# YXHXianYu/RVCP-Real-Time-Path-Tracer

Hardware: AMD Instinct MI355X
Metric: Msamples/sec (pixels*SPP/s) + frame ms, Cornell Box 1024^2 SPP=30 (higher is better)
Workload: dtype f32

## Files before the change

### rvcp-real-time-path-tracer_amd/csrc/rvcp_host.cpp

```cpp
#include <dlfcn.h>
#include <hip/hip_runtime.h>
#include <rccl/rccl.h>

#include <atomic>
#include <cfloat>
#include <cmath>
#include <cstdio>
#include <cstdlib>
#include <chrono>
#include <condition_variable>
#include <cstring>
#include <memory>
#include <exception>
#include <initializer_list>
#include <mutex>
#include <new>
#include <string>
#include <thread>
#include <vector>

#include "../../include/rvcp.h"
#include "rvcp_internal.h"
#include "rvcp_frame_plan.h"
#include "rvcp_jit.h"
// ... 84 lines not shown
        int bvh = 0;
    } capacity[2][2];
    int legacy_capacity = 0;
    uint32_t n_simds = 1024;

    TriRecord *d_tri = nullptr;
    rvcp_face_t *d_faces = nullptr;
    rvcp_vertex_t *d_verts = nullptr;
    MatRecord *d_mats = nullptr;
    FaceShade *d_shade = nullptr;
    LightRecord *d_lights = nullptr;
    rvcp_material_t *d_rawmats = nullptr;
    rvcp_sphere_t *d_spheres = nullptr;
    Bvh4Node *d_bvh_nodes = nullptr;
    TriRecord *d_bvh_tris = nullptr;
    int32_t bvh_root = 0;
    uint32_t bvh_n4 = 0;
    uint32_t bvh_slots = 0;
    int bvh_depth = 0;
    uint32_t bvh_prefix = 0;
    float *d_gamma = nullptr;
    float *d_unorm = nullptr;
    unsigned long long *d_counters = nullptr;
    uint32_t n_faces = 0, n_lights = 0, n_mats = 0, n_verts = 0, n_spheres = 0;
    bool lights_same = false;
    bool rcp_fast = false;
    bool has_metal = false;
    std::shared_ptr<JitKernels> jit[2];
    std::string jit_err;
    int32_t sampling = RVCP_SAMPLING_UNIFORM;
    int32_t jit_sampling[2] = {RVCP_SAMPLING_UNIFORM, -1};
    std::vector<TriRecord> jit_tri;
    bool jit_bvh = false;
    float light_total = 0.0f, light_pdf = 0.0f;
    bool has_scene = false;

    SurfRecord *d_surf = nullptr;
    size_t cap_surf = 0;
    float *d_acc = nullptr;
    size_t cap_acc = 0;
    float *d_cams = nullptr, *h_cams = nullptr;
    uint32_t cap_cams = 0;

    uint32_t *d_rgba = nullptr;
    float *d_lin = nullptr;
    size_t cap_rgba = 0, cap_lin = 0;
    uint32_t *d_pack_rgba = nullptr;
    float *d_pack_lin = nullptr;
    size_t cap_surf_pack = 0;

    Stage stage[N_STAGES];

    float *d_dn[2] = {nullptr, nullptr};
    size_t cap_dn[2] = {0, 0};
    void *d_gbuf = nullptr;
    float *d_dn_in = nullptr, *d_dn_out = nullptr;
    size_t cap_gbuf = 0, cap_dn_in = 0, cap_dn_out = 0;

    float *d_tp_lin[2] = {nullptr, nullptr};
    uint32_t *d_tp_len[2] = {nullptr, nullptr};
    void *d_tp_gbuf[2] = {nullptr, nullptr};
    float *d_tp_cur = nullptr, *d_tp_show = nullptr;
    size_t cap_tp = 0, cap_tp_show = 0;
    History tp_hist;

    float *d_sv_var[2] = {nullptr, nullptr}, *d_sv_tmp[2] = {nullptr, nullptr};
// ... 783 lines not shown
        ctx->bvh_prefix = K;
        if (depth >= kBvhStack) return fail(ctx, RVCP_E_UNSUPPORTED, "BVH deeper than the traversal stack");
        const size_t S = order.size();
        if (S >= (size_t(1) << 26))
            return fail(ctx, RVCP_E_UNSUPPORTED, "BVH leaf slots exceed 2^26 (mesh too large for the leaf encoding)");
        std::vector<TriRecord> btri((10 * S * 4 + sizeof(TriRecord) - 1) / sizeof(TriRecord) + 1);
        float *packed = reinterpret_cast<float *>(btri.data());
        for (size_t j = 0; j < S; j++) {
            if (order[j] == kBvhPadId) continue;
            std::memcpy(packed + 10 * j, &tri[order[j]], 9 * sizeof(float));
            std::memcpy(packed + 10 * j + 9, &order[j], 4);
        }
        ctx->bvh_slots = 0;
        std::vector<Bvh4Node> nodes4;
        int32_t root4 = 0;
        if (bvh4_collapse(nodes, root, nodes4, root4) > kBvhStack)
            return fail(ctx, RVCP_E_UNSUPPORTED, "BVH traversal stack bound exceeded");
        std::vector<Bvh4QNode> q4;
        bvh4_quantize(nodes4, q4);
        std::vector<Bvh4Node> qbuf((q4.size() * sizeof(Bvh4QNode) + sizeof(Bvh4Node) - 1) / sizeof(Bvh4Node));
        if (!q4.empty()) std::memcpy(static_cast<void *>(qbuf.data()), q4.data(), q4.size() * sizeof(Bvh4QNode));
        ctx->bvh_n4 = 0;
        if ((rc = dev_upload<Bvh4Node>(ctx, &ctx->d_bvh_nodes, qbuf.data(), qbuf.size())) ||
            (rc = dev_upload<TriRecord>(ctx, &ctx->d_bvh_tris, btri.data(), btri.size())))
            return rc;
        ctx->bvh_root = root4;
        ctx->bvh_depth = depth;
    }
    ctx->jit[0].reset();
    ctx->jit[1].reset();
    ctx->jit_err.clear();
    ctx->jit_tri.clear();
    ctx->jit_bvh = false;
    ctx->jit_sampling[0] = ctx->sampling;
    ctx->jit_sampling[1] = -1;
    if (bvh_jit) {
        ctx->jit[0] = bvh_jit;
        ctx->jit_tri.assign(tri.begin(), tri.begin() + ctx->bvh_prefix);
        ctx->jit_bvh = true;
    }
    if (ctx->cfg.specialize == RVCP_SPECIALIZE_AUTO && ctx->cfg.accel == RVCP_ACCEL_NONE &&
        n_faces >= 1 && n_faces <= kJitMaxFaces && jit_scene_in_range(tri.data(), n_faces) &&
        !RVCP_KNOB("RVCP_NO_SPECIALIZE")) {
        const bool legacy = ctx->cfg.integrator == RVCP_INTEGRATOR_LEGACY;
        JitSpec spec;
        spec.legacy = legacy;
        spec.sphereless = n_spheres == 0;
        spec.lds_fits = n_spheres <= 64 && n_materials <= 64;
        spec.sampling = ctx->sampling;
        spec.spheres = spheres;
        spec.n_spheres = n_spheres;
        spec.n_materials = n_materials;
        ctx->jit[0] = jit_path_kernels(ctx->device, tri.data(), n_faces, spec, ctx->jit_err);
        HIP_TRY(ctx, hipSetDevice(ctx->device));
        if (!legacy) ctx->jit_tri = tri;
    }
    ctx->rcp_fast = scan_rcp_fast_scene(tri.data(), n_faces);
    ctx->n_faces = n_faces;
    ctx->n_verts = n_vertices;
    ctx->n_mats = n_materials;
    ctx->has_metal = false;
    for (uint32_t i = 0; i < n_materials; i++)
        if (materials[i].ty == 1u) ctx->has_metal = true;
    ctx->n_lights = n_lum_face_ids;
    ctx->lights_same = n_lum_face_ids >= 1;
    for (uint32_t i = 1; i < n_lum_face_ids; i++)
        if (tab.lights[i].face != tab.lights[0].face) ctx->lights_same = false;
    ctx->light_total = total;
    ctx->light_pdf = 1.0f / total;
    ctx->h_rawmats.assign(materials, materials + n_materials);
    ctx->has_scene = true;
    return RVCP_OK;
}

static int impl_upload_scene_file(rvcp_ctx_t *ctx, const char *path, rvcp_camera_t *out_camera)
{
    if (!ctx) return RVCP_E_INVALID;
    SceneFile sf;
    std::string err;
    if (read_scene_file(path, sf, err) != RVCP_OK) return fail(ctx, RVCP_E_INVALID, err);
    const rvcp_lengths_t &L = sf.lengths;
    const int rc = rvcp_upload_scene(ctx, sf.materials.data(), L.materials_len, sf.vertices.data(),
                                     L.vertices_len, sf.faces.data(), L.faces_len, sf.spheres.data(),
                                     L.spheres_len, sf.lum_face_ids.data(), L.luminous_face_id_len,
                                     sf.lum_sphere_ids.data(), L.luminous_sphere_id_len);
    if (rc == RVCP_OK && out_camera) *out_camera = sf.camera;
    return rc;
}

uint32_t rvcp_shard_rows(uint32_t height, uint32_t shard_index, uint32_t shard_count)
{
    if (shard_count == 0 || shard_index >= shard_count) return 0;
    const uint32_t stripes = (height + 7) / 8;
    uint32_t rows = 0;
    for (uint32_t s = shard_index; s < stripes; s += shard_count)
        rows += (s + 1) * 8 <= height ? 8 : height - s * 8;
    return rows;
}

static void jit_for_render(rvcp_ctx_t *ctx, bool map)
{
    ctx->jit_sampling[map] = ctx->sampling;
    if (ctx->jit_tri.empty()) return;
    std::shared_ptr<JitKernels> &jit = ctx->jit[map];
    jit.reset();
    std::string map_err;
    if (!map) ctx->jit_err.clear();
    JitSpec spec;
    spec.bvh = ctx->jit_bvh;
    spec.sampling = ctx->sampling;
    spec.spp_map = map;
    jit = jit_path_kernels(ctx->device, ctx->jit_tri.data(), (uint32_t)ctx->jit_tri.size(), spec,
                           map ? map_err : ctx->jit_err);
    (void)hipSetDevice(ctx->device);
    if (ctx->jit_bvh && jit && (!jit->bvh_path || !jit->bvh_primary)) jit.reset();
}

static FramePlanIn frame_plan_input(const rvcp_ctx_t *ctx, uint32_t n_frames, uint32_t frame_px,
                                    uint32_t stride, uint32_t spp_hint = 0)
{
    const bool cosine = ctx->sampling == RVCP_SAMPLING_COSINE;
    const bool map = spp_hint > 0;
    FramePlanIn in;
    in.integrator = ctx->cfg.integrator;
    in.kernel_variant = ctx->cfg.kernel_variant;
    in.accel = ctx->cfg.accel;
    in.spp = map ? spp_hint : ctx->cfg.spp;
    in.max_bounces = ctx->cfg.max_bounces;
    in.attenuation_stop_eps = ctx->cfg.attenuation_stop_eps;
    in.ray_t_min = ctx->cfg.ray_t_min;
    in.grid_waves_per_simd = ctx->cfg.grid_waves_per_simd;
    in.n_faces = ctx->n_faces;
    in.bvh_prefix = ctx->bvh_prefix;
    in.n_simds = ctx->n_simds;
    const rvcp_ctx::Capacity &cap = ctx->capacity[cosine][map];
    std::memcpy(in.grid_capacity, cap.grid, sizeof(in.grid_capacity));
    in.bvh_capacity = cap.bvh;
    in.legacy_capacity = ctx->legacy_capacity;
    if (const JitKernels *jk = ctx->jit[map].get()) {
        in.module = true;
        in.blocks_per_cu5 = jk->blocks_per_cu5;
        in.blocks_per_cu6 = jk->blocks_per_cu6;
        in.blocks_per_cu_bvh = jk->blocks_per_cu_bvh;
        in.blocks_per_cu_legacy = jk->blocks_per_cu_legacy;
// ... 2999 lines not shown
```

### rvcp-real-time-path-tracer_amd/csrc/rvcp_jit.cpp

```cpp
#include <hip/hip_runtime.h>

#include <dlfcn.h>
#include <sys/stat.h>
#include <unistd.h>

#include <algorithm>
#include <atomic>
#include <cerrno>
#include <cmath>
#include <cstdint>
#include <cstdio>
#include <cstdlib>
#include <cstring>
#include <list>
#include <memory>
#include <mutex>
#include <map>
#include <string>
#include <vector>

#include "rvcp_internal.h"
#include "rvcp_jit.h"
#include "build/rvcp_jit_src.h"

// ... 307 lines not shown
        decl += "    const bool " + pm.name + " = (" + t + " >= tmin) & (" + t + " <= bt" + R + ");\n";
    }
    add(pm.name);
    if (defer) {
        const std::string c = g.prefix + "c";
        accept += "        " + c + " = " + cond + ";\n";
        (inner ? *inner : decl) += "    bool " + c + ";\n";
        pm.pending.emplace_back(c, index);
        return true;
    }
    if (!pm.pending.empty()) {
        const std::string c = g.prefix + "c";
        std::string any = c, best = "best" + R;
        for (const auto &pc : pm.pending) {
            any += " | " + pc.first;
            best = "(" + pc.first + " ? " + std::to_string(pc.second) + " : " + best + ")";
        }
        accept += "        const bool " + c + " = " + cond + ";\n";
        accept += "        if (" + any + ") bt" + R + " = " + t + ";\n";
        if (R != "A")
            accept += "        best" + R + " = " + c + " ? " + std::to_string(index) + " : " + best + ";\n";
        pm.pending.clear();
        return true;
    }
    if (R == "A")
        accept += "        if (" + cond + ") btA = " + t + ";\n";
    else
        accept += "        if (" + cond + ") { bt" + R + " = " + t + "; best" + R + " = " +
                  std::to_string(index) + "; }\n";
    return true;
}

void emit_scan(std::string &out, const TriRecord *tri, uint32_t n, const char *const *rays,
               int n_rays, unsigned opts = 0)
{
    const bool skip_b = (opts & kScanSkipB) != 0, eager = (opts & kScanEagerSplit) != 0;
    const uint32_t N = n * (uint32_t)n_rays;
    std::vector<char> used(N), reused(N);
    {
        std::map<std::string, std::string> seen;
        std::map<std::string, RangeMask> prev;
        for (uint32_t u = 0; u < N; u++) {
            std::string decl, accept;
            bool ru = false;
            used[u] = emit_triangle(decl, accept, tri[u / (uint32_t)n_rays], u / (uint32_t)n_rays,
                                    rays[u % (uint32_t)n_rays], seen, prev, &ru);
            reused[u] = used[u] && ru;
        }
    }
    std::map<std::string, std::string> seen;
    std::map<std::string, RangeMask> prev;
    auto next_used = [&](uint32_t u) {
        uint32_t v = u + (uint32_t)n_rays;
        while (v < N && !used[v]) v += (uint32_t)n_rays;
        return v;
    };
    auto defers = [&](uint32_t u) {
        const uint32_t v = next_used(u);
        return used[u] && v < N && reused[v];
    };
    auto emit_plain = [&](uint32_t u) {
        std::string decl, accept;
        const std::string R(rays[u % (uint32_t)n_rays]);
        const bool defer = defers(u);
        emit_triangle(decl, accept, tri[u / (uint32_t)n_rays], u / (uint32_t)n_rays, R.c_str(),
                      seen, prev, nullptr, defer);
        out += decl;
        if (!used[u]) return;
        out += "    {\n" + accept + "    }\n";
        if (defer) return;
        out += R == "A" ? "    RVCP_SPEC_COMMIT1(btA);\n"
                        : "    RVCP_SPEC_COMMIT(bt" + R + ", best" + R + ");\n";
    };
    if (n_rays == 1) {
        for (uint32_t u = 0; u < N; u++) emit_plain(u);
        return;
    }
    auto emit_split_run = [&](const std::vector<uint32_t> &run, const char *R) {
        std::map<std::string, std::string> inner_seen;
        std::string head, body, accept;
        for (size_t k = 0; k < run.size(); k++) {
            const uint32_t u = run[k];
            const bool defer = k + 1 < run.size();
            std::string decl, inner, acc;
            if (k == 0) {
                emit_triangle(decl, acc, tri[u / 2], u / 2, R, seen, prev, nullptr, defer,
                              &inner, &inner_seen, eager);
                head += decl;
                body += inner;
            } else {
                emit_triangle(decl, acc, tri[u / 2], u / 2, R, inner_seen, prev, nullptr, defer);
                body += decl;
            }
            accept += acc;
        }
        const std::string &mask = prev[R].name;
        const std::string r(R);
        out += head;
        out += "    if (RVCP_SPEC_ANY(" + mask + ")) {\n" + body + "    {\n" + accept + "    }\n    }\n";
        out += r == "A" ? "    RVCP_SPEC_COMMIT1(btA);\n" : "    RVCP_SPEC_COMMIT(bt" + r + ", best" + r + ");\n";
    };
    for (uint32_t i = 0; i < n;) {
        const uint32_t uA = 2 * i;
        if (!used[uA]) {
            emit_plain(uA);
            emit_plain(uA + 1);
            i += 1;
            continue;
        }
        std::vector<uint32_t> run = {uA};
        while (defers(run.back())) run.push_back(next_used(run.back()));
        emit_split_run(run, "A");
        if (skip_b) {
            std::vector<uint32_t> runB;
            for (uint32_t u : run) runB.push_back(u + 1);
            emit_split_run(runB, "B");
        } else {
            for (uint32_t u : run) emit_plain(u + 1);
        }
        i = run.back() / 2 + 1;
    }
}

}
// ... 61 lines not shown
        }
        g.cross(d, e2, s1);
        for (int k = 0; k < 3; k++)
            if (s1[k].kind != Val::kZero && s1[k].mag > 126) return false;
        const Val den = g.dot(s1, e1);
        if (den.kind == Val::kZero) continue;
        if (den.grain == kNoGrain || den.grain < -126 || den.mag > 126) return false;
    }
    return true;
}

bool jit_scene_in_range(const TriRecord *tri, uint32_t n)
{
    for (uint32_t i = 0; i < n; i++)
        for (int k = 0; k < 3; k++)
            if (!(std::fabs(tri[i].v0[k]) <= 0x1p40f) || !(std::fabs(tri[i].e1[k]) <= 0x1p41f) ||
                !(std::fabs(tri[i].e2[k]) <= 0x1p41f))
                return false;
    return true;
}

std::string jit_scan_source(const TriRecord *tri, uint32_t n, unsigned opts)
{
    std::string out = "// generated by rvcp_jit.cpp: the scan of DESIGN.md §4.7 over " +
                      std::to_string(n) + " triangles\n";
    out += "__device__ __forceinline__ void spec_scan1(f3 o, f3 d, float tmin, float &bt, "
           "int &best) {\n";
    static const char *const one[] = {""}, *const two[] = {"A", "B"};
    emit_scan(out, tri, n, one, 1);
    out += "}\n";
    out += "__device__ __forceinline__ void spec_scan2(f3 oA, f3 dA, f3 oB, f3 dB, float tmin, "
           "float &btA, float &btB, int &bestB) {\n";
    emit_scan(out, tri, n, two, 2, opts);
    out += "}\n";
    return out;
}

std::string jit_sphere_source(const rvcp_sphere_t *sph, uint32_t n)
{
    if (n == 0 || n > kJitMaxSpheres || !sph) return std::string();
    std::string out = "// the scene's " + std::to_string(n) + " spheres (rvcp_jit.cpp jit_sphere_source)\n"
                      "#define RVCP_SPEC_SPHERES(X)";
    for (uint32_t i = 0; i < n; i++) {
        out += " \\\n    X(" + std::to_string(i);
        for (float v : {sph[i].center[0], sph[i].center[1], sph[i].center[2], sph[i].radius})
            out += ", " + lit_text(v);
        out += ")";
    }
    return out + "\n";
}

std::string jit_legacy_lds_source(uint32_t n_faces, uint32_t n_spheres, uint32_t n_materials)
{
    auto at_least_1 = [](uint32_t v) { return std::to_string(v ? v : 1u); };
    std::string out = "#define RVCP_LDS_FACES " + at_least_1(n_faces) + "\n#define RVCP_LDS_SPHERES " +
                      at_least_1(n_spheres) + "\n#define RVCP_LDS_MATS " + at_least_1(n_materials) + "\n";
#ifndef RVCP_NO_LDS_PRIMARY
    out += "#define RVCP_LEGACY_LDS_PRIMARY 1\n";
#endif
    return out;
}

namespace {

}

// ... 264 lines not shown
        api.log_size(prog, &ls);
        std::string log(ls, '\0');
        if (ls) api.log(prog, &log[0]);
        err = "hipRTC compile failed: " + log.substr(0, 4000);
        api.destroy(&prog);
        return -1;
    }
    size_t cs = 0;
    api.code_size(prog, &cs);
    code.assign(cs, 0);
    if (cs) api.code(prog, code.data());
    api.destroy(&prog);
    return cs ? 0 : -1;
}

std::string jit_module_source(const TriRecord *tri, uint32_t n, const JitSpec &spec, JitCompile &cc)
{
    cc = JitCompile{};
    cc.legacy = spec.legacy;
    cc.lds_scene = spec.legacy && spec.lds_fits;
#ifndef RVCP_SPHERELESS_LEGACY_WAVES
#define RVCP_SPHERELESS_LEGACY_WAVES 6
#endif
    cc.legacy_waves = spec.legacy && spec.sphereless ? RVCP_SPHERELESS_LEGACY_WAVES : cc.lds_scene ? 5 : 0;
#ifdef RVCP_DEBUG_KNOBS
    if (const char *e = std::getenv("RVCP_JIT_LEGACY_WAVES")) cc.legacy_waves = std::atoi(e);
#endif
    cc.bvh = spec.bvh;
    cc.sampling = spec.sampling;
    cc.spp_map = spec.spp_map;
    std::string key_flags;
    for (const std::string &x : jit_extra_flags()) key_flags += " " + x;
    return jit_scan_source(tri, n, jit_scan_opts()) +
        (spec.legacy ? "// +legacy " + std::to_string(cc.legacy_waves) + (cc.lds_scene ? " lds" : "") + "\n"
#ifndef RVCP_NO_SPHERE_LITERALS
                      + jit_sphere_source(spec.spheres, spec.n_spheres)
#endif
                      + (cc.lds_scene ? jit_legacy_lds_source(n, spec.n_spheres, spec.n_materials) : std::string())
                : std::string()) +
        (key_flags.empty() ? std::string() : "// +flags" + key_flags + "\n") +
        (spec.bvh ? "// +bvh\n" : "") +
        jit_sampling_tag(spec.sampling) + jit_spp_map_tag(spec.spp_map);
}

std::shared_ptr<JitKernels> jit_path_kernels(int device, const TriRecord *tri, uint32_t n,
                                             const JitSpec &spec, std::string &err)
{
    JitCompile cc;
    const std::string scan = jit_module_source(tri, n, spec, cc);
    const bool legacy = spec.legacy, bvh = spec.bvh;
    const uint64_t h = fnv1a(scan);
    std::lock_guard<std::mutex> lock(g_mu);
    for (auto it = g_cache.begin(); it != g_cache.end(); ++it) {
        if (it->device == device && it->hash == h && it->scan == scan) {
            g_cache.splice(g_cache.begin(), g_cache, it);
            return g_cache.front().kernels;
        }
    }
    if (hipSetDevice(device) != hipSuccess) {
        err = "hipSetDevice failed";
        return nullptr;
    }
    auto load = [&](JitKernels &k, const std::vector<char> &code) -> std::string {
        if (hipModuleLoadData(&k.module, code.data()) != hipSuccess) {
            k.module = nullptr;
            return "hipModuleLoadData failed";
// ... 154 lines not shown
{
    return compile_check(tri_records, n, rvcp::JitSpec{}, nullptr, code_bytes, err, err_cap);
}

extern "C" int rvcp_internal_jit_cached_code(const void *tri_records, uint32_t n, int legacy,
                                             int *from_disk, size_t *code_bytes, char *err,
                                             size_t err_cap)
{
    rvcp::JitSpec spec;
    spec.legacy = legacy != 0;
    int disk = 0;
    const int rc = compile_check(tri_records, n, spec, &disk, code_bytes, err, err_cap);
    if (from_disk) *from_disk = disk;
    return rc;
}

extern "C" size_t rvcp_internal_jit_scan_source_opt(const void *tri_records, uint32_t n,
                                                    int opts, char *out, size_t cap)
{
    try {
        return copy_out(rvcp::jit_scan_source(static_cast<const rvcp::TriRecord *>(tri_records), n,
                                              (unsigned)opts), out, cap);
    } catch (...) {
        return 0;
    }
}

extern "C" size_t rvcp_internal_jit_scan_source(const void *tri_records, uint32_t n, char *out,
                                                size_t cap)
{
    return rvcp_internal_jit_scan_source_opt(tri_records, n, 0, out, cap);
}

extern "C" size_t rvcp_internal_jit_sphere_source(const void *spheres, uint32_t n, char *out,
                                                   size_t cap)
{
    try {
        const std::string s = rvcp::jit_sphere_source(static_cast<const rvcp_sphere_t *>(spheres), n);
        if (out && cap > s.size()) std::memcpy(out, s.c_str(), s.size() + 1);
        return s.size();
    } catch (...) {
        return 0;
    }
}

extern "C" size_t rvcp_internal_jit_module_source(const void *tri_records, uint32_t n,
                                                  int sampling, char *out, size_t cap)
{
    return module_source(tri_records, n, hook_spec(sampling), out, cap);
}

extern "C" uint64_t rvcp_internal_jit_module_key_for(const void *tri_records, uint32_t n,
                                                     int sampling)
{
    return module_key(tri_records, n, hook_spec(sampling));
}

extern "C" int rvcp_internal_jit_compile_check_sampling(const void *tri_records, uint32_t n,
                                                         int sampling, size_t *code_bytes,
                                                         char *err, size_t err_cap)
{
    return compile_check(tri_records, n, hook_spec(sampling), nullptr, code_bytes, err, err_cap);
}

extern "C" size_t rvcp_internal_jit_module_source_map(const void *tri_records, uint32_t n,
                                                      int sampling, int spp_map, char *out,
// ... 41 lines not shown
```

### rvcp-real-time-path-tracer_amd/csrc/rvcp_jit.h

```cpp
#pragma once

#include <hip/hip_runtime.h>

#include <memory>
#include <string>
#include <vector>

#include "../../include/rvcp.h"
#include "rvcp_internal.h"

namespace rvcp {

struct JitKernels {
    int device = 0;
    hipModule_t module = nullptr;
    hipFunction_t path5 = nullptr;
    hipFunction_t path6 = nullptr;
    hipFunction_t legacy = nullptr;
    hipFunction_t primary = nullptr;
    hipFunction_t bvh_path = nullptr, bvh_primary = nullptr;
    int blocks_per_cu5 = 0, blocks_per_cu6 = 0, blocks_per_cu_legacy = 0, blocks_per_cu_bvh = 0;
    uint64_t key_hash = 0;
    ~JitKernels();
};

bool jit_scene_in_range(const TriRecord *tri, uint32_t n);
bool scan_rcp_fast_scene(const TriRecord *tri, uint32_t n);
std::vector<std::string> jit_extra_flags();
constexpr unsigned kScanSkipB = 1u, kScanEagerSplit = 2u;
std::string jit_scan_source(const TriRecord *tri, uint32_t n, unsigned opts = 0);
struct JitCompile {
    bool legacy = false;
    int legacy_waves = 0;
    bool lds_scene = false;
    bool bvh = false;
    int sampling = RVCP_SAMPLING_UNIFORM;
    bool spp_map = false;
};
int jit_compile_code(const std::string &scan, std::vector<char> &code, std::string &err,
                     const JitCompile &cc);
int jit_cached_code(const std::string &scan, std::vector<char> &code, std::string &err,
                    const JitCompile &cc, bool *from_disk, bool force_compile);
struct JitSpec {
    bool legacy = false;
    bool sphereless = false;
    bool lds_fits = false;
    bool bvh = false;
    int sampling = RVCP_SAMPLING_UNIFORM;
    bool spp_map = false;
    const rvcp_sphere_t *spheres = nullptr;
    uint32_t n_spheres = 0, n_materials = 64;
};
std::shared_ptr<JitKernels> jit_path_kernels(int device, const TriRecord *tri, uint32_t n,
                                             const JitSpec &spec, std::string &err);
constexpr uint32_t kJitMaxSpheres = 64;
std::string jit_sphere_source(const rvcp_sphere_t *sph, uint32_t n);
std::string jit_legacy_lds_source(uint32_t n_faces, uint32_t n_spheres, uint32_t n_materials);

}
```

### rvcp-real-time-path-tracer_amd/csrc/rvcp_kernels.hip

```cpp
#ifndef __HIPCC_RTC__
#include <hip/hip_runtime.h>
#endif

#ifndef RVCP_SAMPLING
#define RVCP_SAMPLING 0
#endif
#ifndef RVCP_SPP_MAP
#define RVCP_SPP_MAP 0
#endif
#if RVCP_SPP_MAP
#define RVCP_SPP_MAP_PARAM , const uint32_t *__restrict__ spp_map
#define RVCP_SPP_MAP_ARG , spp_map
#else
#define RVCP_SPP_MAP_PARAM
#define RVCP_SPP_MAP_ARG
#endif
#define RVCP_GAMES101_ONLY (RVCP_SAMPLING || RVCP_SPP_MAP)

#include "rvcp_internal.h"
#include "../../include/rvcp.h"
#include "rvcp_sqrt.h"
#include "rvcp_tonemap.h"

#if defined(RVCP_JIT) || !RVCP_GAMES101_ONLY
// ... 185 lines not shown
template <bool FAST = false>
__device__ __forceinline__ bool tri_accept(const TriRecord &T, f3 o, f3 d, float tmin, float bt,
                                           float &t_out) {
    return tri_stage2<FAST>(T, tri_stage1(T, o, d), tmin, bt, t_out);
}
__device__ __forceinline__ float rcp_scan_fast(float den) {
    const float r = __builtin_amdgcn_rcpf(den);
    return __builtin_fmaf(__builtin_fmaf(-den, r, 1.0f), r, r);
}
__device__ __forceinline__ bool dir_grain_ok(f3 d) {
    const uint32_t x = (__float_as_uint(d.x) << 1) - 1u, y = (__float_as_uint(d.y) << 1) - 1u,
                   z = (__float_as_uint(d.z) << 1) - 1u;
    return min(min(x, y), z) >= (0x2B800000u << 1) - 1u;
}
__device__ __forceinline__ bool dir_fast_ok(f3 d) {
    return (((__builtin_fabsf(d.x) + __builtin_fabsf(d.y)) + __builtin_fabsf(d.z)) <= 16.0f) &
           dir_grain_ok(d);
}
#ifdef RVCP_SPEC_SCAN
#define RVCP_F32(bits) __uint_as_float(bits)
#define RVCP_SPEC_COMMIT(t, i) do { asm volatile("" : "+v"(t), "+v"(i)); \
                                    __builtin_amdgcn_sched_barrier(0); } while (0)
#define RVCP_SPEC_COMMIT1(t) do { asm volatile("" : "+v"(t)); \
                                  __builtin_amdgcn_sched_barrier(0); } while (0)
#ifdef RVCP_SPEC_NO_SKIP
#define RVCP_SPEC_ANY(q) ((void)(q), true)
#elif defined(RVCP_SPEC_ISA_SKIP_ALL)
#define RVCP_SPEC_ANY(q) ((void)(q), false)
#else
#define RVCP_SPEC_ANY(q) (__builtin_amdgcn_ballot_w64(q) != 0ull)
#endif
#define RVCP_SPEC_RCP(den) rcp_scan(den)
#define RVCP_SPEC_RCP_FAST(den) rcp_scan_fast(den)
#include RVCP_SPEC_SCAN
__device__ __forceinline__ bool ray_in_range(f3 o, f3 d) {
    return (((__builtin_fabsf(o.x) + __builtin_fabsf(o.y)) + __builtin_fabsf(o.z)) <= 0x1p41f) &
           (((__builtin_fabsf(d.x) + __builtin_fabsf(d.y)) + __builtin_fabsf(d.z)) <= 16.0f) &
           dir_grain_ok(d);
}
#endif
struct TriPartA {
    f3 s, s1;
    float den, n1, m;
};
__device__ __forceinline__ TriPartA tri_stage1a(const TriRecord &T, f3 o, f3 d) {
    TriPartA P;
    P.s = mk(o.x - T.v0[0], o.y - T.v0[1], o.z - T.v0[2]);
    P.s1 = cross(d, ld3(T.e2));
    P.den = dot(P.s1, ld3(T.e1));
    P.n1 = dot(P.s1, P.s);
    P.m = __builtin_fabsf(P.den) * 1.00000095367431640625f;
    return P;
}
__device__ __forceinline__ bool tri_maybe_a(const TriPartA &P) { return __builtin_fabsf(P.n1) <= P.m; }
__device__ __forceinline__ TriPart tri_stage1b(const TriRecord &T, const TriPartA &Pa, f3 d) {
    TriPart P;
    P.s2 = cross(Pa.s, ld3(T.e1));
    P.den = Pa.den;
    P.n1 = Pa.n1;
    P.n2 = dot(P.s2, d);
    return P;
}
__device__ __forceinline__ bool tri_maybe(const TriPart &P) {
    const float m = __builtin_fabsf(P.den) * 1.00000095367431640625f;
    return (__builtin_fabsf(P.n1) <= m) & (__builtin_fabsf(P.n2) <= m);
}

__device__ __forceinline__ bool slab(const float *b, f3 o, f3 inv, float tmin, float bt,
                                     float &tnear) {
    const float x0 = (b[0] - o.x) * inv.x, x1 = (b[3] - o.x) * inv.x;
    const float y0 = (b[1] - o.y) * inv.y, y1 = (b[4] - o.y) * inv.y;
    const float z0 = (b[2] - o.z) * inv.z, z1 = (b[5] - o.z) * inv.z;
// ... 2124 lines not shown
            for (uint32_t off = R >> 1; off >= 1; off >>= 1) {
                const float ot = __shfl_xor(bt, (int)off);
                const int ob = __shfl_xor(best, (int)off);
                if (ot < bt || (ot == bt && ob > best)) { bt = ot; best = ob; }
            }
            const int srcA = hasA ? (int)(rank_in(mA) * R) : (int)lane;
            const int srcB = hasB ? (int)((na + rank_in(mB)) * R) : (int)lane;
            const float tA_ = __shfl(bt, srcA), tB_ = __shfl(bt, srcB);
            const int iA_ = __shfl(best, srcA), iB_ = __shfl(best, srcB);
            if (hasA) { btA = tA_; bestA = iA_; }
            if (hasB) { btB = tB_; bestB = iB_; }
        } else if (!TILED && wave_active && nr <= (uint32_t)kWave) {
            float4 *rows = compact_lds + wv * (2 * kWave);
            if (hasA) {
                const uint32_t j = rank_in(mA);
                rows[2 * j] = make_float4(a_o.x, a_o.y, a_o.z, 0.0f);
                rows[2 * j + 1] = make_float4(a_d.x, a_d.y, a_d.z, 0.0f);
            }
            if (hasB) {
                const uint32_t j = na + rank_in(mB);
                rows[2 * j] = make_float4(b_o.x, b_o.y, b_o.z, 0.0f);
                rows[2 * j + 1] = make_float4(b_d.x, b_d.y, b_d.z, 0.0f);
            }
            __builtin_amdgcn_fence(__ATOMIC_RELEASE, "wavefront");
            __builtin_amdgcn_wave_barrier();
            __builtin_amdgcn_fence(__ATOMIC_ACQUIRE, "wavefront");
            uint32_t lane_r;
            asm volatile("v_mbcnt_lo_u32_b32 %0, -1, 0\n\tv_mbcnt_hi_u32_b32 %0, -1, %0"
                         : "=v"(lane_r));
            const float4 ro = rows[2 * lane_r], rd = rows[2 * lane_r + 1];
            const f3 o = mk(ro.x, ro.y, ro.z), d = mk(rd.x, rd.y, rd.z);
            float bt = A.t_max;
            int best = -1;
#ifdef RVCP_SPEC_SCAN
            if (!__any(lane_r < nr && !ray_in_range(o, d))) {
                spec_scan1(o, d, A.t_min, bt, best);
            } else
#endif
            if (A.rcp_fast && !__any(lane_r < nr && !dir_fast_ok(d)))
                scan_generic1<true>(tri, A.n_faces, o, d, A.t_min, bt, best);
            else
                scan_generic1<false>(tri, A.n_faces, o, d, A.t_min, bt, best);
            __builtin_amdgcn_fence(__ATOMIC_RELEASE, "wavefront");
            __builtin_amdgcn_wave_barrier();
            __builtin_amdgcn_fence(__ATOMIC_ACQUIRE, "wavefront");
            rows[2 * lane_r] = make_float4(bt, __int_as_float(best), 0.0f, 0.0f);
            __builtin_amdgcn_fence(__ATOMIC_RELEASE, "wavefront");
            __builtin_amdgcn_wave_barrier();
            __builtin_amdgcn_fence(__ATOMIC_ACQUIRE, "wavefront");
            if (hasA) {
                const float4 r = rows[2 * rank_in(mA)];
                btA = r.x;
                bestA = __float_as_int(r.y);
            }
            if (hasB) {
                const float4 r = rows[2 * (na + rank_in(mB))];
                btB = r.x;
                bestB = __float_as_int(r.y);
            }
        } else {
#ifdef RVCP_SPEC_SCAN
            if (!__any((hasA && !ray_in_range(a_o, a_d)) || (hasB && !ray_in_range(b_o, b_d)))) {
                if (!hasA) btA = -1.0f;
                spec_scan2(a_o, a_d, b_o, b_d, A.t_min, btA, btB, bestB);
            } else
#endif
            {
            if (!SINGLE && !hasA) btA = -1.0f;
            if (A.rcp_fast && !__any((hasA && !dir_fast_ok(a_d)) || (hasB && !dir_fast_ok(b_d))))
                scan_generic2<true, SINGLE>(tri, A.n_faces, a_o, a_d, b_o, b_d, A.t_min, btA, bestA, btB, bestB);
            else
                scan_generic2<false, SINGLE>(tri, A.n_faces, a_o, a_d, b_o, b_d, A.t_min, btA, bestA, btB, bestB);
            }
            if (!SINGLE) {
                bestA = btA != A.t_max ? 0 : -1;
                if (__builtin_expect(__any(hasA && btA == A.t_max), 0)) {
                    btA = A.t_max;
                    bestA = -1;
                    for (uint32_t i = 0; i < A.n_faces; ++i) {
                        float tA;
                        if (tri_accept(tri[i], a_o, a_d, A.t_min, btA, tA)) { btA = tA; bestA = (int)i; }
                    }
                }
            }
        }

        if (SINGLE && !hasA) {
            btB = btA;
            bestB = bestA;
        }
        RC_END(1);
        RC_BEGIN(3);

        if (LDS_STATE) col = st_get3(13);
// ... 1321 lines not shown
```

Before: 11650.

## Add grouped JIT scan that culls connected face groups with bounding boxes

```diff
diff --git a/rvcp-real-time-path-tracer_amd/csrc/rvcp_host.cpp b/rvcp-real-time-path-tracer_amd/csrc/rvcp_host.cpp
--- a/rvcp-real-time-path-tracer_amd/csrc/rvcp_host.cpp
+++ b/rvcp-real-time-path-tracer_amd/csrc/rvcp_host.cpp
@@ -140,6 +140,7 @@
     int32_t jit_sampling[2] = {RVCP_SAMPLING_UNIFORM, -1};
     std::vector<TriRecord> jit_tri;
     bool jit_bvh = false;
+    uint64_t jit_lum = 0;
     float light_total = 0.0f, light_pdf = 0.0f;
     bool has_scene = false;
 
@@ -989,6 +990,7 @@
     ctx->jit_err.clear();
     ctx->jit_tri.clear();
     ctx->jit_bvh = false;
+    ctx->jit_lum = 0;
     ctx->jit_sampling[0] = ctx->sampling;
     ctx->jit_sampling[1] = -1;
     if (bvh_jit) {
@@ -1008,6 +1010,9 @@
         spec.spheres = spheres;
         spec.n_spheres = n_spheres;
         spec.n_materials = n_materials;
+        for (uint32_t i = 0; i < n_lum_face_ids; i++)
+            if (tab.lights[i].face < 64u) spec.lum_mask |= 1ull << tab.lights[i].face;
+        ctx->jit_lum = spec.lum_mask;
         ctx->jit[0] = jit_path_kernels(ctx->device, tri.data(), n_faces, spec, ctx->jit_err);
         HIP_TRY(ctx, hipSetDevice(ctx->device));
         if (!legacy) ctx->jit_tri = tri;
@@ -1067,6 +1072,7 @@
     spec.bvh = ctx->jit_bvh;
     spec.sampling = ctx->sampling;
     spec.spp_map = map;
+    spec.lum_mask = ctx->jit_lum;
     jit = jit_path_kernels(ctx->device, ctx->jit_tri.data(), (uint32_t)ctx->jit_tri.size(), spec,
                            map ? map_err : ctx->jit_err);
     (void)hipSetDevice(ctx->device);
diff --git a/rvcp-real-time-path-tracer_amd/csrc/rvcp_jit.cpp b/rvcp-real-time-path-tracer_amd/csrc/rvcp_jit.cpp
--- a/rvcp-real-time-path-tracer_amd/csrc/rvcp_jit.cpp
+++ b/rvcp-real-time-path-tracer_amd/csrc/rvcp_jit.cpp
@@ -363,10 +363,11 @@
 }
 
 void emit_scan(std::string &out, const TriRecord *tri, uint32_t n, const char *const *rays,
-               int n_rays, unsigned opts = 0)
+               int n_rays, unsigned opts = 0, const uint32_t *ids = nullptr)
 {
     const bool skip_b = (opts & kScanSkipB) != 0, eager = (opts & kScanEagerSplit) != 0;
     const uint32_t N = n * (uint32_t)n_rays;
+    auto face = [&](uint32_t k) { return ids ? ids[k] : k; };
     std::vector<char> used(N), reused(N);
     {
         std::map<std::string, std::string> seen;
@@ -374,7 +375,7 @@
         for (uint32_t u = 0; u < N; u++) {
             std::string decl, accept;
             bool ru = false;
-            used[u] = emit_triangle(decl, accept, tri[u / (uint32_t)n_rays], u / (uint32_t)n_rays,
+            used[u] = emit_triangle(decl, accept, tri[face(u / (uint32_t)n_rays)], face(u / (uint32_t)n_rays),
                                     rays[u % (uint32_t)n_rays], seen, prev, &ru);
             reused[u] = used[u] && ru;
         }
@@ -394,8 +395,8 @@
         std::string decl, accept;
         const std::string R(rays[u % (uint32_t)n_rays]);
         const bool defer = defers(u);
-        emit_triangle(decl, accept, tri[u / (uint32_t)n_rays], u / (uint32_t)n_rays, R.c_str(),
-                      seen, prev, nullptr, defer);
+        emit_triangle(decl, accept, tri[face(u / (uint32_t)n_rays)], face(u / (uint32_t)n_rays),
+                      R.c_str(), seen, prev, nullptr, defer);
         out += decl;
         if (!used[u]) return;
         out += "    {\n" + accept + "    }\n";
@@ -415,12 +416,12 @@
             const bool defer = k + 1 < run.size();
             std::string decl, inner, acc;
             if (k == 0) {
-                emit_triangle(decl, acc, tri[u / 2], u / 2, R, seen, prev, nullptr, defer,
+                emit_triangle(decl, acc, tri[face(u / 2)], face(u / 2), R, seen, prev, nullptr, defer,
                               &inner, &inner_seen, eager);
                 head += decl;
                 body += inner;
             } else {
-                emit_triangle(decl, acc, tri[u / 2], u / 2, R, inner_seen, prev, nullptr, defer);
+                emit_triangle(decl, acc, tri[face(u / 2)], face(u / 2), R, inner_seen, prev, nullptr, defer);
                 body += decl;
             }
             accept += acc;
@@ -548,6 +549,202 @@
     out += "__device__ __forceinline__ void spec_scan2(f3 oA, f3 dA, f3 oB, f3 dB, float tmin, "
            "float &btA, float &btB, int &bestB) {\n";
     emit_scan(out, tri, n, two, 2, opts);
+    out += "}\n";
+    return out;
+}
+
+namespace {
+constexpr uint32_t kMaxGroups = 4;
+constexpr uint32_t kGroupMinFaces = 6;
+constexpr uint32_t kGroupMaxNormals = 6;
+constexpr double kGroupPad = 1.0 / 64;
+constexpr double kGroupHeight = 0.25;
+constexpr double kGroupCoord = 1024.0;
+constexpr double kGroupOrigin = 1.5;
+constexpr double kGroupNormalCos = 1.0 - 1e-9;
+constexpr float kGroupParallel = 0x1p-7f;
+
+float round_down(double x)
+{
+    float f = (float)x;
+    return (double)f > x ? std::nextafterf(f, -INFINITY) : f;
+}
+float round_up(double x)
+{
+    float f = (float)x;
+    return (double)f < x ? std::nextafterf(f, INFINITY) : f;
+}
+void face_points(const TriRecord &T, double p[3][3])
+{
+    for (int k = 0; k < 3; k++) {
+        p[0][k] = T.v0[k];
+        p[1][k] = (double)T.v0[k] + (double)T.e1[k];
+        p[2][k] = (double)T.v0[k] + (double)T.e2[k];
+    }
+}
+}
+
+ScanGroups jit_scan_groups(const TriRecord *tri, uint32_t n, uint64_t lum_mask)
+{
+    ScanGroups G;
+    G.group_of.assign(n, -1);
+    if (n == 0 || n > 64) return G;
+    double lo[3] = {INFINITY, INFINITY, INFINITY}, hi[3] = {-INFINITY, -INFINITY, -INFINITY}, amax = 0.0;
+    for (uint32_t i = 0; i < n; i++) {
+        double p[3][3];
+        face_points(tri[i], p);
+        for (int v = 0; v < 3; v++)
+            for (int k = 0; k < 3; k++) {
+                if (!std::isfinite(p[v][k])) return G;
+                lo[k] = std::min(lo[k], p[v][k]);
+                hi[k] = std::max(hi[k], p[v][k]);
+                amax = std::max(amax, std::fabs(p[v][k]));
+            }
+    }
+    const double L = std::max(hi[0] - lo[0], std::max(hi[1] - lo[1], hi[2] - lo[2]));
+    if (!(L > 0.0) || !(amax <= kGroupCoord * L) || !(L <= 0x1p40)) return G;
+    const double pad = kGroupPad * L;
+    auto area_of = [](const double a[3], const double b[3], double grow) {
+        const double x = b[0] - a[0] + 2 * grow, y = b[1] - a[1] + 2 * grow, z = b[2] - a[2] + 2 * grow;
+        return 2.0 * (x * y + y * z + z * x);
+    };
+    const double scene_area = area_of(lo, hi, 0.0);
+    std::vector<uint32_t> parent(n);
+    for (uint32_t i = 0; i < n; i++) parent[i] = i;
+    auto find = [&](uint32_t x) {
+        while (parent[x] != x) x = parent[x] = parent[parent[x]];
+        return x;
+    };
+    std::map<std::vector<uint32_t>, uint32_t> first;
+    for (uint32_t i = 0; i < n; i++) {
+        for (int v = 0; v < 3; v++) {
+            std::vector<uint32_t> key(3);
+            for (int k = 0; k < 3; k++) {
+                float c = v == 0 ? tri[i].v0[k] : tri[i].v0[k] + (v == 1 ? tri[i].e1[k] : tri[i].e2[k]);
+                if (c == 0.0f) c = 0.0f;
+                std::memcpy(&key[k], &c, 4);
+            }
+            const auto it = first.find(key);
+            if (it == first.end()) first[key] = i;
+            else parent[find(i)] = find(it->second);
+        }
+    }
+    for (uint32_t root = 0; root < n && G.groups.size() < kMaxGroups; root++) {
+        if (find(root) != root) continue;
+        ScanGroup g;
+        double glo[3] = {INFINITY, INFINITY, INFINITY}, ghi[3] = {-INFINITY, -INFINITY, -INFINITY};
+        bool ok = true;
+        for (uint32_t i = 0; i < n && ok; i++) {
+            if (find(i) != root) continue;
+            g.faces.push_back(i);
+            if ((lum_mask >> i) & 1ull) ok = false;
+            double p[3][3], e[3][3], len2[3], nrm[3];
+            face_points(tri[i], p);
+            for (int k = 0; k < 3; k++) {
+                e[0][k] = p[1][k] - p[0][k];
+                e[1][k] = p[2][k] - p[0][k];
+                e[2][k] = p[2][k] - p[1][k];
+            }
+            for (int j = 0; j < 3; j++) len2[j] = e[j][0] * e[j][0] + e[j][1] * e[j][1] + e[j][2] * e[j][2];
+            nrm[0] = e[0][1] * e[1][2] - e[0][2] * e[1][1];
+            nrm[1] = e[0][2] * e[1][0] - e[0][0] * e[1][2];
+            nrm[2] = e[0][0] * e[1][1] - e[0][1] * e[1][0];
+            const double area2 = std::sqrt(nrm[0] * nrm[0] + nrm[1] * nrm[1] + nrm[2] * nrm[2]);
+            const double longest2 = std::max(len2[0], std::max(len2[1], len2[2]));
+            if (!(longest2 > 0.0) || !(area2 >= kGroupHeight * longest2)) { ok = false; break; }
+            for (int k = 0; k < 3; k++) nrm[k] /= area2;
+            bool known = false;
+            for (const auto &r : g.normals)
+                if (std::fabs(r[0] * nrm[0] + r[1] * nrm[1] + r[2] * nrm[2]) >= kGroupNormalCos) known = true;
+            if (!known) g.normals.push_back({nrm[0], nrm[1], nrm[2]});
+            for (int v = 0; v < 3; v++)
+                for (int k = 0; k < 3; k++) {
+                    glo[k] = std::min(glo[k], p[v][k]);
+                    ghi[k] = std::max(ghi[k], p[v][k]);
+                }
+        }
+        if (!ok || g.faces.size() < kGroupMinFaces || g.normals.size() > kGroupMaxNormals) continue;
+        if (!(area_of(glo, ghi, pad) <= 0.25 * scene_area)) continue;
+        for (int k = 0; k < 3; k++) {
+            g.lo[k] = round_down(glo[k] - pad);
+            g.hi[k] = round_up(ghi[k] + pad);
+        }
+        for (uint32_t f : g.faces) G.group_of[f] = (int)G.groups.size();
+        G.groups.push_back(g);
+    }
+    for (int k = 0; k < 3; k++) {
+        G.centre[k] = (float)(0.5 * (lo[k] + hi[k]));
+        G.reach[k] = round_down(kGroupOrigin * L);
+    }
+    return G;
+}
+
+std::string jit_groups_source(const TriRecord *tri, uint32_t n, uint64_t lum_mask, unsigned opts)
+{
+    const ScanGroups G = jit_scan_groups(tri, n, lum_mask);
+    if (G.groups.empty()) return std::string();
+    static const char *const one[] = {""}, *const two[] = {"A", "B"};
+    std::string out = "// the grouped scan (rvcp_jit.cpp jit_groups_source, DESIGN.md §4.7): " +
+                      std::to_string(G.groups.size()) + " face groups\n#define RVCP_SPEC_GROUPS " +
+                      std::to_string(G.groups.size()) + "\n";
+    out += "__device__ __forceinline__ bool spec_group_origin_ok(f3 o) {\n    return ";
+    for (int k = 0; k < 3; k++) {
+        const std::string c = std::string("o.") + "xyz"[k];
+        out += std::string(k ? " &\n           " : "") + "(__builtin_fabsf(" + c + " - " + lit_text(G.centre[k]) +
+               ") <= " + lit_text(G.reach[k]) + ")";
+    }
+    out += ";\n}\n";
+    out += "__device__ __forceinline__ unsigned spec_group_reach(f3 o, f3 d, float tmin, float bt) {\n"
+           "    const float ix = RVCP_SPEC_BOX_RCP(d.x), iy = RVCP_SPEC_BOX_RCP(d.y), iz = RVCP_SPEC_BOX_RCP(d.z);\n"
+           "    const float dn = ((__builtin_fabsf(d.x) + __builtin_fabsf(d.y)) + __builtin_fabsf(d.z)) * " +
+           lit_text(kGroupParallel) + ";\n    unsigned m = 0u;\n";
+    for (size_t gi = 0; gi < G.groups.size(); gi++) {
+        const ScanGroup &g = G.groups[gi];
+        out += "    {\n";
+        for (int k = 0; k < 3; k++) {
+            const std::string c(1, "xyz"[k]);
+            out += "        const float a" + c + " = (" + lit_text(g.lo[k]) + " - o." + c + ") * i" + c +
+                   ", b" + c + " = (" + lit_text(g.hi[k]) + " - o." + c + ") * i" + c + ";\n";
+        }
+        out += "        const float tn = __builtin_fmaxf(__builtin_fmaxf(__builtin_fminf(ax, bx), __builtin_fminf(ay, by)), "
+               "__builtin_fmaxf(__builtin_fminf(az, bz), tmin));\n"
+               "        const float tf = __builtin_fminf(__builtin_fminf(__builtin_fmaxf(ax, bx), __builtin_fmaxf(ay, by)), "
+               "__builtin_fminf(__builtin_fmaxf(az, bz), bt));\n"
+               "        bool r = !(tn > tf);\n";
+        for (const auto &nr : g.normals) {
+            std::string e;
+            for (int k = 0; k < 3; k++) {
+                const float c = (float)nr[k];
+                if (c == 0.0f) continue;
+                const std::string dk = std::string("d.") + "xyz"[k];
+                e = e.empty() ? dk + " * " + lit_text(c)
+                              : "__builtin_fmaf(" + dk + ", " + lit_text(c) + ", " + e + ")";
+            }
+            if (e.empty()) e = "0.0f";
+            out += "        r |= __builtin_fabsf(" + e + ") < dn;\n";
+        }
+        out += "        m |= r ? " + std::to_string(1u << gi) + "u : 0u;\n    }\n";
+    }
+    out += "    return m;\n}\n";
+    std::vector<uint32_t> always;
+    for (uint32_t i = 0; i < n; i++)
+        if (G.group_of[i] < 0) always.push_back(i);
+    out += "__device__ __forceinline__ void spec_always1(f3 o, f3 d, float tmin, float &bt, int &best) {\n";
+    emit_scan(out, tri, (uint32_t)always.size(), one, 1, 0, always.data());
+    out += "}\n__device__ __forceinline__ void spec_always2(f3 oA, f3 dA, f3 oB, f3 dB, float tmin, "
+           "float &btA, float &btB, int &bestB) {\n";
+    emit_scan(out, tri, (uint32_t)always.size(), two, 2, opts, always.data());
+    out += "}\n";
+    for (size_t gi = 0; gi < G.groups.size(); gi++) {
+        out += "__device__ __forceinline__ void spec_group_scan" + std::to_string(gi) +
+               "(f3 o, f3 d, float tmin, float &bt, int &best) {\n";
+        emit_scan(out, tri, (uint32_t)G.groups[gi].faces.size(), one, 1, 0, G.groups[gi].faces.data());
+        out += "}\n";
+    }
+    out += "__device__ __forceinline__ void spec_group_scan(int g, f3 o, f3 d, float tmin, float &bt, int &best) {\n";
+    for (size_t gi = 0; gi < G.groups.size(); gi++)
+        out += "    if (g == " + std::to_string(gi) + ") spec_group_scan" + std::to_string(gi) +
+               "(o, d, tmin, bt, best);\n";
     out += "}\n";
     return out;
 }
@@ -878,6 +1075,7 @@
     std::string key_flags;
     for (const std::string &x : jit_extra_flags()) key_flags += " " + x;
     return jit_scan_source(tri, n, jit_scan_opts()) +
+        (spec.legacy || spec.bvh ? std::string() : jit_groups_source(tri, n, spec.lum_mask, jit_scan_opts())) +
         (spec.legacy ? "// +legacy " + std::to_string(cc.legacy_waves) + (cc.lds_scene ? " lds" : "") + "\n"
 #ifndef RVCP_NO_SPHERE_LITERALS
                       + jit_sphere_source(spec.spheres, spec.n_spheres)
@@ -1098,6 +1296,35 @@
     return rvcp_internal_jit_scan_source_opt(tri_records, n, 0, out, cap);
 }
 
+extern "C" size_t rvcp_internal_jit_groups_source(const void *tri_records, uint32_t n,
+                                                  uint64_t lum_mask, char *out, size_t cap)
+{
+    try {
+        return copy_out(rvcp::jit_groups_source(static_cast<const rvcp::TriRecord *>(tri_records), n,
+                                                lum_mask), out, cap);
+    } catch (...) {
+        return 0;
+    }
+}
+
+extern "C" int rvcp_internal_jit_groups(const void *tri_records, uint32_t n, uint64_t lum_mask,
+                                        int32_t *group_of, float *box)
+{
+    try {
+        const rvcp::ScanGroups G =
+            rvcp::jit_scan_groups(static_cast<const rvcp::TriRecord *>(tri_records), n, lum_mask);
+        for (uint32_t i = 0; group_of && i < n; i++) group_of[i] = G.group_of[i];
+        for (size_t g = 0; box && g < G.groups.size(); g++)
+            for (int k = 0; k < 3; k++) {
+                box[6 * g + k] = G.groups[g].lo[k];
+                box[6 * g + 3 + k] = G.groups[g].hi[k];
+            }
+        return (int)G.groups.size();
+    } catch (...) {
+        return -1;
+    }
+}
+
 extern "C" size_t rvcp_internal_jit_sphere_source(const void *spheres, uint32_t n, char *out,
                                                    size_t cap)
 {
diff --git a/rvcp-real-time-path-tracer_amd/csrc/rvcp_jit.h b/rvcp-real-time-path-tracer_amd/csrc/rvcp_jit.h
--- a/rvcp-real-time-path-tracer_amd/csrc/rvcp_jit.h
+++ b/rvcp-real-time-path-tracer_amd/csrc/rvcp_jit.h
@@ -2,6 +2,7 @@
 
 #include <hip/hip_runtime.h>
 
+#include <array>
 #include <memory>
 #include <string>
 #include <vector>
@@ -29,6 +30,18 @@
 std::vector<std::string> jit_extra_flags();
 constexpr unsigned kScanSkipB = 1u, kScanEagerSplit = 2u;
 std::string jit_scan_source(const TriRecord *tri, uint32_t n, unsigned opts = 0);
+struct ScanGroup {
+    std::vector<uint32_t> faces;
+    float lo[3], hi[3];
+    std::vector<std::array<double, 3>> normals;
+};
+struct ScanGroups {
+    std::vector<int> group_of;
+    std::vector<ScanGroup> groups;
+    float centre[3] = {0, 0, 0}, reach[3] = {0, 0, 0};
+};
+ScanGroups jit_scan_groups(const TriRecord *tri, uint32_t n, uint64_t lum_mask);
+std::string jit_groups_source(const TriRecord *tri, uint32_t n, uint64_t lum_mask, unsigned opts = 0);
 struct JitCompile {
     bool legacy = false;
     int legacy_waves = 0;
@@ -50,6 +63,7 @@
     bool spp_map = false;
     const rvcp_sphere_t *spheres = nullptr;
     uint32_t n_spheres = 0, n_materials = 64;
+    uint64_t lum_mask = 0;
 };
 std::shared_ptr<JitKernels> jit_path_kernels(int device, const TriRecord *tri, uint32_t n,
                                              const JitSpec &spec, std::string &err);
diff --git a/rvcp-real-time-path-tracer_amd/csrc/rvcp_kernels.hip b/rvcp-real-time-path-tracer_amd/csrc/rvcp_kernels.hip
--- a/rvcp-real-time-path-tracer_amd/csrc/rvcp_kernels.hip
+++ b/rvcp-real-time-path-tracer_amd/csrc/rvcp_kernels.hip
@@ -241,12 +241,84 @@
 #endif
 #define RVCP_SPEC_RCP(den) rcp_scan(den)
 #define RVCP_SPEC_RCP_FAST(den) rcp_scan_fast(den)
+#define RVCP_SPEC_BOX_RCP(x) __builtin_amdgcn_rcpf(x)
 #include RVCP_SPEC_SCAN
 __device__ __forceinline__ bool ray_in_range(f3 o, f3 d) {
     return (((__builtin_fabsf(o.x) + __builtin_fabsf(o.y)) + __builtin_fabsf(o.z)) <= 0x1p41f) &
            (((__builtin_fabsf(d.x) + __builtin_fabsf(d.y)) + __builtin_fabsf(d.z)) <= 16.0f) &
            dir_grain_ok(d);
 }
+#ifdef RVCP_SPEC_GROUPS
+__device__ __forceinline__ bool spec_ray_ok(f3 o, f3 d) {
+    return ray_in_range(o, d) & spec_group_origin_ok(o);
+}
+__device__ __forceinline__ void spec_group_pass(float4 *rows, float tmin, bool hasA, f3 a_o, f3 a_d,
+                                                float &btA, bool hasB, f3 b_o, f3 b_d, float &btB,
+                                                int &bestB) {
+    const uint32_t rA = hasA ? spec_group_reach(a_o, a_d, tmin, btA) : 0u;
+    const uint32_t rB = hasB ? spec_group_reach(b_o, b_d, tmin, btB) : 0u;
+    if (__builtin_amdgcn_ballot_w64((rA | rB) != 0u) == 0ull) return;
+    uint64_t m[2 * RVCP_SPEC_GROUPS];
+    uint32_t base[2 * RVCP_SPEC_GROUPS], total = 0u;
+#pragma unroll
+    for (int g = 0; g < RVCP_SPEC_GROUPS; g++) {
+        m[2 * g] = __builtin_amdgcn_ballot_w64(((rA >> g) & 1u) != 0u);
+        base[2 * g] = total;
+        total += (uint32_t)__builtin_popcountll(m[2 * g]);
+        m[2 * g + 1] = __builtin_amdgcn_ballot_w64(((rB >> g) & 1u) != 0u);
+        base[2 * g + 1] = total;
+        total += (uint32_t)__builtin_popcountll(m[2 * g + 1]);
+    }
+    for (uint32_t p0 = 0u; p0 < total; p0 += (uint32_t)kWave) {
+        __builtin_amdgcn_fence(__ATOMIC_RELEASE, "wavefront");
+        __builtin_amdgcn_wave_barrier();
+        __builtin_amdgcn_fence(__ATOMIC_ACQUIRE, "wavefront");
+#pragma unroll
+        for (int g = 0; g < RVCP_SPEC_GROUPS; g++) {
+            const uint32_t jA = base[2 * g] + rank_in(m[2 * g]) - p0;
+            if (((rA >> g) & 1u) != 0u && jA < (uint32_t)kWave) {
+                rows[2 * jA] = make_float4(a_o.x, a_o.y, a_o.z, btA);
+                rows[2 * jA + 1] = make_float4(a_d.x, a_d.y, a_d.z, __int_as_float(g));
+            }
+            const uint32_t jB = base[2 * g + 1] + rank_in(m[2 * g + 1]) - p0;
+            if (((rB >> g) & 1u) != 0u && jB < (uint32_t)kWave) {
+                rows[2 * jB] = make_float4(b_o.x, b_o.y, b_o.z, btB);
+                rows[2 * jB + 1] = make_float4(b_d.x, b_d.y, b_d.z, __int_as_float(g));
+            }
+        }
+        __builtin_amdgcn_fence(__ATOMIC_RELEASE, "wavefront");
+        __builtin_amdgcn_wave_barrier();
+        __builtin_amdgcn_fence(__ATOMIC_ACQUIRE, "wavefront");
+        const uint32_t lane_r = lane_id();
+        const float4 ro = rows[2 * lane_r], rd = rows[2 * lane_r + 1];
+        float bt = ro.w;
+        int best = -1;
+        if (lane_r < total - p0)
+            spec_group_scan(__float_as_int(rd.w), mk(ro.x, ro.y, ro.z), mk(rd.x, rd.y, rd.z), tmin, bt, best);
+        __builtin_amdgcn_fence(__ATOMIC_RELEASE, "wavefront");
+        __builtin_amdgcn_wave_barrier();
+        __builtin_amdgcn_fence(__ATOMIC_ACQUIRE, "wavefront");
+        rows[2 * lane_r] = make_float4(bt, __int_as_float(best), 0.0f, 0.0f);
+        __builtin_amdgcn_fence(__ATOMIC_RELEASE, "wavefront");
+        __builtin_amdgcn_wave_barrier();
+        __builtin_amdgcn_fence(__ATOMIC_ACQUIRE, "wavefront");
+#pragma unroll
+        for (int g = 0; g < RVCP_SPEC_GROUPS; g++) {
+            const uint32_t jA = base[2 * g] + rank_in(m[2 * g]) - p0;
+            if (((rA >> g) & 1u) != 0u && jA < (uint32_t)kWave) {
+                const float4 r = rows[2 * jA];
+                if (__float_as_int(r.y) >= 0 && r.x < btA) btA = r.x;
+            }
+            const uint32_t jB = base[2 * g + 1] + rank_in(m[2 * g + 1]) - p0;
+            if (((rB >> g) & 1u) != 0u && jB < (uint32_t)kWave) {
+                const float4 r = rows[2 * jB];
+                const int ob = __float_as_int(r.y);
+                if (ob >= 0 && (r.x < btB || (r.x == btB && ob > bestB))) { btB = r.x; bestB = ob; }
+            }
+        }
+    }
+}
+#endif
 #endif
 struct TriPartA {
     f3 s, s1;
@@ -2437,7 +2509,13 @@
             const f3 o = mk(ro.x, ro.y, ro.z), d = mk(rd.x, rd.y, rd.z);
             float bt = A.t_max;
             int best = -1;
-#ifdef RVCP_SPEC_SCAN
+#ifdef RVCP_SPEC_GROUPS
+            if (!__any(lane_r < nr && !spec_ray_ok(o, d))) {
+                spec_always1(o, d, A.t_min, bt, best);
+                float no_bt = -1.0f;
+                spec_group_pass(rows, A.t_min, false, o, d, no_bt, lane_r < nr, o, d, bt, best);
+            } else
+#elif defined(RVCP_SPEC_SCAN)
             if (!__any(lane_r < nr && !ray_in_range(o, d))) {
                 spec_scan1(o, d, A.t_min, bt, best);
             } else
@@ -2464,7 +2542,15 @@
                 bestB = __float_as_int(r.y);
             }
         } else {
-#ifdef RVCP_SPEC_SCAN
+#ifdef RVCP_SPEC_GROUPS
+            if (!TILED && !BVH &&
+                !__any((hasA && !spec_ray_ok(a_o, a_d)) || (hasB && !spec_ray_ok(b_o, b_d)))) {
+                if (!hasA) btA = -1.0f;
+                spec_always2(a_o, a_d, b_o, b_d, A.t_min, btA, btB, bestB);
+                spec_group_pass(compact_lds + wv * (2 * kWave), A.t_min, hasA, a_o, a_d, btA, hasB,
+                                b_o, b_d, btB, bestB);
+            } else
+#elif defined(RVCP_SPEC_SCAN)
             if (!__any((hasA && !ray_in_range(a_o, a_d)) || (hasB && !ray_in_range(b_o, b_d)))) {
                 if (!hasA) btA = -1.0f;
                 spec_scan2(a_o, a_d, b_o, b_d, A.t_min, btA, btB, bestB);
```

Result: faster. 11840 (median of 6 runs) (+1.6%).
